# henkkagee/fpc-diffrend

Hardware: AMD Instinct MI355X
Metric: fit-loop frames/sec (9-view 1080p) (higher is better)
Workload: dtype f32; 1 GPU; cfg3: 9-view 1920x1080, K=150 blendshapes, T=30000 triangles, 32 frames/GPU/step (288 images), textured C=1 + antialias fwd/bwd, Adam on weights+pose+texture; frames_per_gpu=32, views=9, triangles=30000, parallelism=one GPU, no collective

## Files before the change

fpc_diffrend_amd/_lib.py:

```python
import ctypes
import os
import subprocess

_HERE = os.path.dirname(os.path.abspath(__file__))
LIB_PATH = os.environ.get("FPCDR_LIB_PATH") or os.path.join(_HERE, "libfpcdr.so")
TWOCALL_LIB_PATH = os.environ.get("FPCDR_TWOCALL_LIB_PATH") or os.path.join(_HERE, "libfpcdr_twocall.so")
CSRC = os.path.join(_HERE, "csrc")

MAX_ATTR = 32
MAX_MIP = 16
LOSS_SLOTS = 256
OCC_BIN = 32
ABI_VERSION = 16

FILTER = {'nearest': 0, 'linear': 1, 'linear-mipmap-nearest': 2, 'linear-mipmap-linear': 3}
BOUNDARY = {'wrap': 0, 'clamp': 1, 'zero': 2}

_p = ctypes.c_void_p
_i = ctypes.c_int32


class RasterizeFwd(ctypes.Structure):
    _fields_ = [("pos", _p), ("tri", _p), ("B", _i), ("V", _i), ("T", _i), ("H", _i), ("W", _i), ("scratch", _p),
                ("rast", _p), ("rast_db", _p), ("hint", _p), ("ranges", _p)]
# ... 99 lines not shown
                ("bg", ctypes.c_float), ("color_scale", ctypes.c_float), ("grad_scale", ctypes.c_float), ("eps", ctypes.c_float),
                ("radius", _i), ("taps", ctypes.c_float * 64), ("tmp", _p), ("stats", _p), ("d", _p), ("pq", _p), ("p", _p),
                ("loss_sum", _p), ("grad_color", _p)]


ROBUST_KIND = {'l2': 0, 'charbonnier': 1, 'geman_mcclure': 2}


class RobustLoss(ctypes.Structure):
    _fields_ = [("color", _p), ("rast", _p), ("ref", _p), ("B", _i), ("H", _i), ("W", _i), ("C", _i),
                ("bg", ctypes.c_float), ("color_scale", ctypes.c_float), ("grad_scale", ctypes.c_float), ("kind", _i),
                ("inv_c", ctypes.c_float), ("w_outside", ctypes.c_float), ("sat", _i), ("mask", _p), ("face_w", _p), ("T", _i),
                ("sums", _p), ("grad_color", _p)]


WSUM_SLOTS = 32


class ObjectiveWeighted(ctypes.Structure):
    _fields_ = [("base", Objective), ("kind", _i), ("inv_c", ctypes.c_float), ("w_outside", ctypes.c_float), ("sat", _i),
                ("T_weights", _i), ("mask", _p), ("face_w", _p), ("wsum", _p)]


ADAM_MAX_TENSORS = 16


class AdamTensor(ctypes.Structure):
    _fields_ = [("param", _p), ("grad", _p), ("exp_avg", _p), ("exp_avg_sq", _p), ("n", ctypes.c_int64),
                ("step_size", ctypes.c_float), ("bc2_sqrt", ctypes.c_float), ("renorm", _i), ("table_row", _i),
                ("step", _i), ("lr", ctypes.c_float)]


class AdamParams(ctypes.Structure):
    _fields_ = [("n_tensors", _i), ("beta1", ctypes.c_float), ("beta2", ctypes.c_float), ("eps", ctypes.c_float),
                ("one_minus_beta1", ctypes.c_float), ("one_minus_beta2", ctypes.c_float), ("t", AdamTensor * ADAM_MAX_TENSORS),
                ("step_table", _p), ("skip_flag", _p), ("skipped", _p), ("lr_skip_gain", ctypes.c_double),
                ("skipped_per_tensor", _p), ("beta1_f64", ctypes.c_double), ("beta2_f64", ctypes.c_double)]


_sz = ctypes.c_size_t
_int = ctypes.c_int
SYMBOLS = {
    "fpcdr_abi_version": (_int, []),
    "fpcdr_last_error": (ctypes.c_char_p, []),
    "fpcdr_rasterize_scratch_bytes": (_sz, [_i, _i]),
    "fpcdr_rasterize_fwd": (_int, [ctypes.POINTER(RasterizeFwd), _p]),
    "fpcdr_rasterize_bwd": (_int, [ctypes.POINTER(RasterizeBwd), _p]),
    "fpcdr_occ_bytes": (_sz, [_i, _i, _i]),
    "fpcdr_cmask_bytes": (_sz, [_i, _i, _i]),
    "fpcdr_objective_cmask_bytes": (_sz, [_i, _i, _i]),
    "fpcdr_ref_bg_sumsq": (_int, [_p, ctypes.c_int64, ctypes.c_int64, ctypes.c_float, _p, _p]),
    "fpcdr_objective_value": (_int, [_p, _i, _p, ctypes.c_double, ctypes.c_double, _p, _p]),
    "fpcdr_idplane_bytes": (_sz, [_i, _i, _i]),
    "fpcdr_binlist_bytes": (_sz, [_i, _i, _i]),
    "fpcdr_objective_fwd": (_int, [ctypes.POINTER(Objective), _p]),
    "fpcdr_silhouette_bits": (_int, [_p, _p, _p, _i, _i, _i, _i, _i, _p, _p]),
    "fpcdr_interpolate_fwd": (_int, [ctypes.POINTER(InterpolateFwd), _p]),
    "fpcdr_interpolate_bwd": (_int, [ctypes.POINTER(InterpolateBwd), _p]),
    "fpcdr_mip_downsample": (_int, [_p, _p, _i, _i, _i, _i, _p]),
    "fpcdr_mip_downsample_bwd": (_int, [_p, _p, _i, _i, _i, _i, _p]),
    "fpcdr_texture_fwd": (_int, [ctypes.POINTER(TextureFwd), _p]),
    "fpcdr_texture_bwd": (_int, [ctypes.POINTER(TextureBwd), _p]),
    "fpcdr_topology_scratch_bytes": (_sz, [_i]),
    "fpcdr_topology_build": (_int, [_p, _i, _p, _p, _p]),
    "fpcdr_antialias_flags_bytes": (_sz, [_i, _i, _i]),
    "fpcdr_antialias_fwd": (_int, [ctypes.POINTER(AntialiasFwd), _p]),
    "fpcdr_antialias_bwd": (_int, [ctypes.POINTER(AntialiasBwd), _p]),
    "fpcdr_transform_clip_fwd": (_int, [_p, _p, _p, _i, _i, _i, _p]),
    "fpcdr_transform_clip_bwd": (_int, [_p, _p, _p, _p, _p, _i, _i, _i, _p]),
    "fpcdr_mvp_fwd": (_int, [_p, _p, _p, _p, _p, _p, _p, _i, _i, _p]),
    "fpcdr_mvp_bwd": (_int, [_p, _p, _p, _p, _p, _p, _p, _p, _p, _p, _p, _i, _i, _p]),
    "fpcdr_mvp_fwd_indexed": (_int, [_p, _p, _p, _p, _p, _p, _p, _p, _p, _p, _i, _i, _p]),
    "fpcdr_mvp_bwd_indexed": (_int, [_p, _p, _p, _p, _p, _p, _p, _p, _p, _p, _p, _p, _p, _p, _i, _i, _p]),
    "fpcdr_laplacian_gather": (_int, [_p, _p, _p, _p, _i, _i, _i, _i, _p]),
    "fpcdr_laplacian_penalty_fwd": (_int, [_p, _p, _p, _p, _p, _p, _p, ctypes.c_float, _i, _i, _i, _p]),
    "fpcdr_laplacian_penalty_bwd": (_int, [_p, _p, _p, _p, _p, _p, ctypes.c_float, _i, _i, _i, _p]),
    "fpcdr_laplacian_penalty_rest_fwd": (_int, [_p, _p, _p, _p, _p, _p, _p, _p, ctypes.c_float, _i, _i, _i, _p]),
    "fpcdr_stretch_penalty": (_int, [_p, _p, _p, ctypes.c_float, _p, _p, _p, _p, ctypes.c_float, _i, _i, _i, _i, _p]),
    "fpcdr_bend_penalty": (_int, [_p, _p, _p, _p, _p, _p, _p, _p, _p, ctypes.c_float, _i, _i, _i, _i, _p]),
    "fpcdr_motion_penalty": (_int, [_p, _p, _p, ctypes.c_float, _i, _p, _p, _p, _p, ctypes.c_float, _i, _i, _p]),
    "fpcdr_tex_prior": (_int, [_p, _p, _p, _p, ctypes.c_float, ctypes.c_float, ctypes.c_float, _p, _p, _p, _p, _i, _i, _i, _p]),
    "fpcdr_blend_fwd": (_int, [_p, _p, _p, _p, _i, _i, _i, _p]),
    "fpcdr_blend_bwd_w": (_int, [_p, _p, _p, _i, _i, _i, _p]),
    "fpcdr_blend_bwd_basis": (_int, [_p, _p, _p, _i, _i, _i, _p]),
    "fpcdr_rig_weights_fwd": (_int, [_p, _p, _p, _i, _i, _i, _i, _i, _p, _p]),
    "fpcdr_rig_weights_bwd": (_int, [_p, _p, _p, _i, _p, _i, _i, _i, _i, _p, _p, _p]),
    "fpcdr_pixel_loss": (_int, [ctypes.POINTER(PixelLoss), _p]),
    "fpcdr_blur_loss_scratch_bytes": (_sz, [_i, _i, _i, _i]),
    "fpcdr_blur_loss": (_int, [ctypes.POINTER(BlurLoss), _p]),
    "fpcdr_norm_loss_scratch_bytes": (_sz, [_i, _i, _i, _i]),
    "fpcdr_norm_loss": (_int, [ctypes.POINTER(NormLoss), _p]),
    "fpcdr_robust_loss": (_int, [ctypes.POINTER(RobustLoss), _p]),
    "fpcdr_objective_weighted_fwd": (_int, [ctypes.POINTER(ObjectiveWeighted), _p]),
    "fpcdr_ref_bg_wsum": (_int, [_p, _p, ctypes.c_int64, ctypes.c_int64, ctypes.c_float, _i, ctypes.c_float, ctypes.c_float, _i, _p, _p]),
    "fpcdr_adam_step": (_int, [ctypes.POINTER(AdamParams), _p]),
    "fpcdr_undistort_u8": (_int, [_p, _p, _p, ctypes.c_int64, _i, _i, _i, _i, _i, _p]),
    "fpcdr_compare_u8": (_int, [_p, _int, ctypes.c_float, _p, _p, _p, ctypes.c_int64, _i, _i, _i, _i, _i, _i, _p]),
    "fpcdr_overlay_u8": (_int, [_p, _int, ctypes.c_float, _p, _p, _p, _p, ctypes.c_int64, _i, _i, _int, _int, ctypes.c_float,
                                ctypes.c_uint32, _int, _p]),
    "fpcdr_bake_accumulate_u8": (_int, [_p, _p, _p, _p, ctypes.c_int64, _i, _i, _i, _i, _i, _i, _i, _p]),
    "fpcdr_bake_resolve": (_int, [_p, _p, _p, _i, _i, ctypes.c_double, ctypes.c_uint64, _p]),
    "fpcdr_bake_dilate": (_int, [_p, _p, _p, _p, _i, _i, _p]),
    "fpcdr_downsample_u8": (_int, [_p, _p, ctypes.c_int64, _i, _i, _i, _p]),
}

SYMBOLS_TWOCALL = {
    "fpcdr_render_fwd": (_int, [ctypes.POINTER(RenderFwd), _p]),
    "fpcdr_render_bwd": (_int, [ctypes.POINTER(RenderBwd), _p]),
    "fpcdr_aa_loss_fwd": (_int, [ctypes.POINTER(AaLossFwd), _p]),
    "fpcdr_render_loss_fwd": (_int, [ctypes.POINTER(RenderFwd), ctypes.POINTER(AaLossFwd), _p, _p]),
    "fpcdr_render_aa_bwd": (_int, [ctypes.POINTER(RenderAaBwd), _p]),
}

_lib = None
_lib_twocall = None


def build(force=False):
    cmd = ["make", "-s", "-C", CSRC, "-j8"] + (["-B"] if force else [])
    subprocess.check_call(cmd)
    return LIB_PATH


def load():
    global _lib
    if _lib is not None:
        return _lib
    if not os.path.exists(LIB_PATH):
        raise RuntimeError(
            f"{LIB_PATH} not found: the HIP extension is not built. Run `python -c 'import __graft_entry__ as g; "
            f"g.build()'` (or `make -C {CSRC}`). There is no CPU fallback for the raster ops.")
    import torch
    hip_rt = os.path.join(os.path.dirname(torch.__file__), "lib", "libamdhip64.so")
    if os.path.exists(hip_rt):
        ctypes.CDLL(hip_rt, mode=ctypes.RTLD_GLOBAL)
    lib = ctypes.CDLL(LIB_PATH)
    for name, (res, args) in SYMBOLS.items():
        fn = getattr(lib, name)
        fn.restype = res
        fn.argtypes = args
    ver = lib.fpcdr_abi_version()
    if ver != ABI_VERSION:
        raise RuntimeError(f"libfpcdr.so ABI version {ver} != binding {ABI_VERSION}; rebuild the extension")
    _lib = lib
    return lib


def load_twocall():
    global _lib_twocall
    if _lib_twocall is not None:
        return _lib_twocall
    load()
    if not os.path.exists(TWOCALL_LIB_PATH):
        raise RuntimeError(f"{TWOCALL_LIB_PATH} not found: run `make -C {CSRC}` (or __graft_entry__.build()). The two-call form of the "
                           "pixel objective and ops.render_textured live in this second library; there is no fallback.")
    lib = ctypes.CDLL(TWOCALL_LIB_PATH)
    for name, (res, args) in list(SYMBOLS.items()) + list(SYMBOLS_TWOCALL.items()):
        fn = getattr(lib, name)
        fn.restype = res
        fn.argtypes = args
    if lib.fpcdr_abi_version() != ABI_VERSION:
        raise RuntimeError(f"libfpcdr_twocall.so ABI version {lib.fpcdr_abi_version()} != binding {ABI_VERSION}; rebuild the extension")
    _lib_twocall = lib
    return lib


# ... 40 lines not shown
```

fpc_diffrend_amd/csrc/blend.hip:

```cpp
#include "common.h"

namespace {

typedef float f32x16 __attribute__((ext_vector_type(16)));

constexpr int KC = 64;

__device__ __forceinline__ int acc_row(int r, int lane) { return (r & 3) + 8 * (r >> 2) + 4 * (lane >> 5); }

__global__ void __launch_bounds__(256) k_blend_fwd(const float *__restrict__ v_base, const float *__restrict__ Bmat,
                                                   const float *__restrict__ w, float *__restrict__ out, int M, int K, int F) {
    const int lane = threadIdx.x & 63, wave = threadIdx.x >> 6;
    const int tile = blockIdx.x * 4 + wave;
    const int i0 = tile * 32;
    if (i0 >= M) return;
    const int col = lane & 31, h = lane >> 5;
    const int row = min(i0 + col, M - 1);
    const float *brow = Bmat + (size_t)row * K;
    for (int f0 = 0; f0 < F; f0 += 32) {
        const int fr = min(f0 + col, F - 1);
        const float *wrow = w + (size_t)fr * K;
        f32x16 acc = {0, 0, 0, 0, 0, 0, 0, 0, 0, 0, 0, 0, 0, 0, 0, 0};
        if ((K & 1) == 0) {
            for (int kc = 0; kc < K; kc += 2 * KC) {
// ... 107 lines not shown
                s_w[r * KP + K + e - r * np] = 0.0f;
            }
        }
        store_tile(s_w, vw4);
        __syncthreads();
        f32x16 acc = {0, 0, 0, 0, 0, 0, 0, 0, 0, 0, 0, 0, 0, 0, 0, 0};
        const float *pa = s_w + col * KP + kbase, *pb = s_b + col * KP + kbase;
        for (int s = 0; s < kh; s += 4) {
            const float4 a = *reinterpret_cast<const float4 *>(pa + s);
            const float4 b = *reinterpret_cast<const float4 *>(pb + s);
            acc = __builtin_amdgcn_mfma_f32_32x32x2f32(a.x, b.x, acc, 0, 0, 0);
            acc = __builtin_amdgcn_mfma_f32_32x32x2f32(a.y, b.y, acc, 0, 0, 0);
            acc = __builtin_amdgcn_mfma_f32_32x32x2f32(a.z, b.z, acc, 0, 0, 0);
            acc = __builtin_amdgcn_mfma_f32_32x32x2f32(a.w, b.w, acc, 0, 0, 0);
        }
        __syncthreads();
        if (wave > 0) {
#pragma unroll
            for (int r = 0; r < 16; ++r) s_red[((wave - 1) * 16 + r) * 64 + lane] = acc[r];
        }
        __syncthreads();
        if (wave == 0) {
            const int i = i0 + col;
            const float vb = (v_base && i < M) ? v_base[i] : 0.0f;
#pragma unroll
            for (int r = 0; r < 16; ++r) {
                const float v = acc[r] + s_red[r * 64 + lane] + s_red[(16 + r) * 64 + lane] + s_red[(32 + r) * 64 + lane];
                const int f = f0 + acc_row(r, lane);
                if (f < F && i < M) out[(size_t)f * M + i] = v + vb;
            }
        }
    }
}

#define FPCDR_BLEND_SLAB 512
constexpr int SLAB = FPCDR_BLEND_SLAB;
__global__ void __launch_bounds__(256) k_blend_bwd_w(const float *__restrict__ Bmat, const float *__restrict__ gout,
                                                     float *__restrict__ grad_w, int M, int K, int F) {
    const int lane = threadIdx.x & 63, wave = threadIdx.x >> 6;
    const int col = lane & 31, h = lane >> 5;
    const int k0 = blockIdx.x * 32, f0 = blockIdx.z * 32;
    const int kk = k0 + col, fr = min(f0 + col, F - 1);
    const int rows_per_wave = SLAB / 4, rows_per_half = rows_per_wave / 2;
    const int base = blockIdx.y * SLAB + wave * rows_per_wave + h * rows_per_half;
    const float *grow = gout + (size_t)fr * M;
    f32x16 acc = {0, 0, 0, 0, 0, 0, 0, 0, 0, 0, 0, 0, 0, 0, 0, 0};
    if ((M & 1) == 0) {
#pragma unroll 8
        for (int s = 0; s < rows_per_half; s += 2) {
            const int i = base + s;
            const bool ok = i < M;
            const float2 a = ok ? *reinterpret_cast<const float2 *>(grow + i) : make_float2(0.f, 0.f);
            const float b0 = (ok && kk < K) ? Bmat[(size_t)i * K + kk] : 0.0f;
            const float b1 = (ok && kk < K) ? Bmat[(size_t)(i + 1) * K + kk] : 0.0f;
            acc = __builtin_amdgcn_mfma_f32_32x32x2f32(a.x, b0, acc, 0, 0, 0);
            acc = __builtin_amdgcn_mfma_f32_32x32x2f32(a.y, b1, acc, 0, 0, 0);
        }
    } else {
#pragma unroll 8
        for (int s = 0; s < rows_per_half; ++s) {
            const int i = base + s;
            const bool ok = i < M;
            const float a = ok ? grow[i] : 0.0f;
            const float b = (ok && kk < K) ? Bmat[(size_t)i * K + kk] : 0.0f;
            acc = __builtin_amdgcn_mfma_f32_32x32x2f32(a, b, acc, 0, 0, 0);
        }
    }
    __shared__ float s_red[3][16][64];
    if (wave > 0) {
#pragma unroll
        for (int r = 0; r < 16; ++r) s_red[wave - 1][r][lane] = acc[r];
    }
    __syncthreads();
    if (wave == 0 && kk < K) {
#pragma unroll
        for (int r = 0; r < 16; ++r) {
            const int f = f0 + acc_row(r, lane);
            const float v = acc[r] + s_red[0][r][lane] + s_red[1][r][lane] + s_red[2][r][lane];
            if (f < F && v != 0.0f) atomicAdd(grad_w + (size_t)f * K + kk, v);
        }
    }
}

__global__ void __launch_bounds__(256) k_blend_bwd_basis(const float *__restrict__ w, const float *__restrict__ gout,
                                                         float *__restrict__ grad_B, int M, int K, int F) {
    const int lane = threadIdx.x & 63, wave = threadIdx.x >> 6;
    const int col = lane & 31, h = lane >> 5;
    const int i0 = (blockIdx.x * 4 + wave) * 32, k0 = blockIdx.y * 32;
    if (i0 >= M) return;
    const int ii = min(i0 + col, M - 1), kk = min(k0 + col, K - 1);
    f32x16 acc = {0, 0, 0, 0, 0, 0, 0, 0, 0, 0, 0, 0, 0, 0, 0, 0};
    const int half = (F + 1) / 2;
    for (int s = 0; s < half; ++s) {
        const int f = h * half + s;
        const bool ok = f < F && (h == 0 ? s < half : true);
        const float a = ok ? gout[(size_t)f * M + ii] : 0.0f;
        const float b = ok ? w[(size_t)f * K + kk] : 0.0f;
        acc = __builtin_amdgcn_mfma_f32_32x32x2f32(a, b, acc, 0, 0, 0);
    }
    const int k = k0 + col;
    if (k < K) {
#pragma unroll
        for (int r = 0; r < 16; ++r) {
            const int i = i0 + acc_row(r, lane);
            if (i < M) grad_B[(size_t)i * K + k] = acc[r];
        }
    }
}

__device__ __forceinline__ int rig_col(const int64_t *__restrict__ cols, int col0, int fb, int Fc) {
    if (!cols) return col0 + fb;
    long long c = cols[fb];
    if (c < 0) c += Fc;
    return (c >= 0 && c < Fc) ? (int)c : -1;
}

__global__ void __launch_bounds__(256) k_rig_weights_fwd(const float *__restrict__ mi, const float *__restrict__ maps,
                                                         const int64_t *__restrict__ cols, int col0, int K, int Fr, int Fc, int Fb,
                                                         float *__restrict__ w) {
    const int idx = blockIdx.x * 256 + threadIdx.x;
    if (idx >= Fb * K) return;
    const int fb = idx / K, k = idx - fb * K;
    const int c = rig_col(cols, col0, fb, Fc);
    if (c < 0) { w[idx] = __int_as_float(0x7fc00000); return; }
    float s = 0.0f;
#pragma unroll 8
    for (int f = 0; f < Fr; ++f) s += mi[(size_t)k * Fr + f] * maps[(size_t)f * Fc + c];
    w[idx] = s;
}

__global__ void __launch_bounds__(256) k_rig_weights_bwd(const float *__restrict__ mi, const float *__restrict__ maps,
                                                         const int64_t *__restrict__ cols, int col0, const float *__restrict__ g_w,
                                                         int K, int Fr, int Fc, int Fb, float *__restrict__ g_mi, float *__restrict__ g_maps) {
    const int lane = threadIdx.x & 63;
    int idx = blockIdx.x * 4 + (threadIdx.x >> 6);
    if (idx < K * Fr) {
        if (!g_mi) return;
        const int k = idx / Fr, f = idx - k * Fr;
        float s = 0.0f;
        for (int fb = lane; fb < Fb; fb += 64) {
            const int c = rig_col(cols, col0, fb, Fc);
            if (c >= 0) s += g_w[(size_t)fb * K + k] * maps[(size_t)f * Fc + c];
        }
        s = wave_sum_dpp(s);
        if (lane == 0) g_mi[idx] = s;
        return;
    }
    idx -= K * Fr;
    if (idx >= Fr * Fc || !g_maps) return;
    const int f = idx / Fc, c = idx - f * Fc;
    float s = 0.0f;
    for (int fb = 0; fb < Fb; ++fb) {
        if (rig_col(cols, col0, fb, Fc) != c) continue;
        for (int k = lane; k < K; k += 64) s += mi[(size_t)k * Fr + f] * g_w[(size_t)fb * K + k];
    }
    s = wave_sum_dpp(s);
    if (lane == 0) g_maps[idx] = s;
}

}

extern "C" int fpcdr_blend_fwd(const float *v_base, const float *Bmat, const float *w, float *out, int32_t M, int32_t K,
                               int32_t F, void *stream) {
    FPCDR_REQUIRE(Bmat && w && out, "null pointer");
    FPCDR_REQUIRE(M > 0 && K > 0 && F > 0, "sizes must be positive");
    if (K <= LDS_KMAX && ((size_t)Bmat & 15) == 0 && ((size_t)w & 15) == 0) {
        const int KQ = (K + 31) / 32 * 32;
        const size_t tile = (size_t)32 * (KQ + 4);
        const size_t lds = (tile + (tile > 3 * 16 * 64 ? tile : (size_t)3 * 16 * 64)) * sizeof(float);
        hipLaunchKernelGGL(k_blend_fwd_lds, dim3(fpcdr_cdiv(M, TM)), dim3(256), lds, (hipStream_t)stream, v_base, Bmat, w, out, M, K,
                           F, KQ);
        FPCDR_CHECK_LAUNCH();
        return FPCDR_OK;
    }
    hipLaunchKernelGGL(k_blend_fwd, dim3(fpcdr_cdiv(fpcdr_cdiv(M, 32), 4)), dim3(256), 0, (hipStream_t)stream, v_base, Bmat, w,
                       out, M, K, F);
    FPCDR_CHECK_LAUNCH();
    return FPCDR_OK;
}

extern "C" int fpcdr_blend_bwd_w(const float *Bmat, const float *grad_out, float *grad_w, int32_t M, int32_t K, int32_t F,
                                 void *stream) {
    FPCDR_REQUIRE(Bmat && grad_out && grad_w, "null pointer");
    FPCDR_REQUIRE(M > 0 && K > 0 && F > 0, "sizes must be positive");
    FPCDR_REQUIRE(fpcdr_cdiv(M, SLAB) <= 65535 && fpcdr_cdiv(F, 32) <= 65535, "problem too large for one launch");
    dim3 grid(fpcdr_cdiv(K, 32), fpcdr_cdiv(M, SLAB), fpcdr_cdiv(F, 32));
    hipLaunchKernelGGL(k_blend_bwd_w, grid, dim3(256), 0, (hipStream_t)stream, Bmat, grad_out, grad_w, M, K, F);
    FPCDR_CHECK_LAUNCH();
    return FPCDR_OK;
}

extern "C" int fpcdr_blend_bwd_basis(const float *w, const float *grad_out, float *grad_B, int32_t M, int32_t K, int32_t F,
                                     void *stream) {
    FPCDR_REQUIRE(w && grad_out && grad_B, "null pointer");
    FPCDR_REQUIRE(M > 0 && K > 0 && F > 0, "sizes must be positive");
    FPCDR_REQUIRE(fpcdr_cdiv(K, 32) <= 65535, "K too large for one launch");
    dim3 grid(fpcdr_cdiv(fpcdr_cdiv(M, 32), 4), fpcdr_cdiv(K, 32));
    hipLaunchKernelGGL(k_blend_bwd_basis, grid, dim3(256), 0, (hipStream_t)stream, w, grad_out, grad_B, M, K, F);
    FPCDR_CHECK_LAUNCH();
    return FPCDR_OK;
}

extern "C" int fpcdr_rig_weights_fwd(const float *mi, const float *maps, const int64_t *cols, int32_t col0, int32_t K, int32_t Fr, int32_t Fc,
                                     int32_t Fb, float *w, void *stream) {
    FPCDR_REQUIRE(mi && maps && w, "null pointer");
    FPCDR_REQUIRE(K > 0 && Fr > 0 && Fc > 0 && Fb > 0 && (long long)Fb * K < (1ll << 30), "bad sizes");
    FPCDR_REQUIRE(cols || (col0 >= 0 && col0 + Fb <= Fc), "column range outside maps");
    hipLaunchKernelGGL(k_rig_weights_fwd, dim3(fpcdr_cdiv(Fb * K, 256)), dim3(256), 0, (hipStream_t)stream, mi, maps, cols, col0, K, Fr, Fc, Fb, w);
    FPCDR_CHECK_LAUNCH();
    return FPCDR_OK;
}

extern "C" int fpcdr_rig_weights_bwd(const float *mi, const float *maps, const int64_t *cols, int32_t col0, const float *grad_w, int32_t K,
                                     int32_t Fr, int32_t Fc, int32_t Fb, float *grad_mi, float *grad_maps, void *stream) {
    FPCDR_REQUIRE(mi && maps && grad_w, "null pointer");
    FPCDR_REQUIRE(K > 0 && Fr > 0 && Fc > 0 && Fb > 0 && (long long)Fb * K < (1ll << 30) && (long long)K * Fr + (long long)Fr * Fc < (1ll << 30),
                  "bad sizes");
    FPCDR_REQUIRE(cols || (col0 >= 0 && col0 + Fb <= Fc), "column range outside maps");
    hipLaunchKernelGGL(k_rig_weights_bwd, dim3(fpcdr_cdiv(K * Fr + Fr * Fc, 4)), dim3(256), 0, (hipStream_t)stream, mi, maps, cols, col0,
                       grad_w, K, Fr, Fc, Fb, grad_mi, grad_maps);
    FPCDR_CHECK_LAUNCH();
    return FPCDR_OK;
}
```

fpc_diffrend_amd/fit.py:

```python
import ctypes
import json
import math
import os
import time
from dataclasses import dataclass
from typing import Optional, Sequence, Tuple

import numpy as np
import torch

from . import _lib, camera
from . import ops as dr
from .mesh_reg import (MeshTopology, RestShape, _check_item_weights, _uniform_laplacian, bend_penalty, check_motion_options,
                       hinge_incidence, hinge_rest_cs, hinge_vertices, laplacian_penalty, mesh_edge_loss, mesh_laplacian_smoothing,
                       mesh_normal_consistency, motion_inv_scale, motion_penalty, rest_edge_lengths, stretch_penalty)
from .ops import _ptr, _stream
from .tex_prior import chart_map, check_tex_prior_options, load_texel_weights, tex_prior_inv_scale, texture_prior

BACKGROUND = 45.0 / 255.0



class ZeroPool:

    def __init__(self, buf=None):
        self.buf, self.off = buf, 0

    def zeros(self, shape, device):
        n = int(np.prod(shape))
        if self.buf is not None and self.buf.device == device and self.off + n <= self.buf.numel():
            v = self.buf[self.off:self.off + n].view(shape)
            self.off += (n + 3) // 4 * 4
            return v
        return torch.zeros(shape, dtype=torch.float32, device=device)


def _pool_zeros(pool, shape, device):
    return pool.zeros(shape, device) if pool is not None else torch.zeros(shape, dtype=torch.float32, device=device)


class _blend_func(torch.autograd.Function):

    @staticmethod
    def forward(ctx, v_base, Bmat, w, pool=None):
        lib = _lib.load()
        M, K = Bmat.shape
        F = w.shape[0]
        out = torch.empty(F, M, dtype=torch.float32, device=w.device)
        _lib.call("fpcdr_blend_fwd", _ptr(v_base), _ptr(Bmat), _ptr(w), _ptr(out), M, K, F, _stream())
        ctx.save_for_backward(Bmat, w)
        ctx.pool = pool
        return out

    @staticmethod
    def backward(ctx, g):
        lib = _lib.load()
        Bmat, w = ctx.saved_tensors
        M, K = Bmat.shape
        F = w.shape[0]
        g = g.contiguous()
        g_vb = g.sum(dim=0) if ctx.needs_input_grad[0] else None
        g_B = None
        if ctx.needs_input_grad[1]:
            g_B = torch.empty_like(Bmat)
            _lib.call("fpcdr_blend_bwd_basis", _ptr(w), _ptr(g), _ptr(g_B), M, K, F, _stream())
        g_w = None
        if ctx.needs_input_grad[2]:
            g_w = _pool_zeros(ctx.pool, tuple(w.shape), w.device)
            _lib.call("fpcdr_blend_bwd_w", _ptr(Bmat), _ptr(g), _ptr(g_w), M, K, F, _stream())
        return g_vb, g_B, g_w, None


class _transform_clip_func(torch.autograd.Function):

    @staticmethod
    def forward(ctx, mvp, verts, pool=None):
        B, F, V = mvp.shape[0], verts.shape[0], verts.shape[1]
        out = torch.empty(B, V, 4, dtype=torch.float32, device=verts.device)
        _lib.call("fpcdr_transform_clip_fwd", _ptr(mvp), _ptr(verts), _ptr(out), F, B // F, V, _stream())
        ctx.save_for_backward(mvp, verts)
        ctx.pool = pool
        return out

    @staticmethod
    def backward(ctx, g):
        mvp, verts = ctx.saved_tensors
        B, F, V = mvp.shape[0], verts.shape[0], verts.shape[1]
        g = g.contiguous()
        g_mvp = _pool_zeros(ctx.pool, tuple(mvp.shape), mvp.device) if ctx.needs_input_grad[0] else None
        g_verts = torch.empty_like(verts) if ctx.needs_input_grad[1] else None
        _lib.call("fpcdr_transform_clip_bwd", _ptr(mvp), _ptr(verts), _ptr(g), _ptr(g_verts), _ptr(g_mvp), F, B // F, V, _stream())
        return g_mvp, g_verts, None


class _rig_weights_func(torch.autograd.Function):

    @staticmethod
    def forward(ctx, mi, maps, ids, validate=True):
        K, Fr = mi.shape
        Fc = maps.shape[1]
        if isinstance(ids, slice):
            lo, hi, step = ids.indices(Fc)
            assert step == 1
            cols, col0, Fb = None, lo, hi - lo
        else:
            cols, col0, Fb = ids.to(torch.int64).contiguous(), 0, int(ids.shape[0])
            if validate and Fb and bool(((cols < -Fc) | (cols >= Fc)).any()):
                raise IndexError(f"rig_weights: frame index out of range for {Fc} columns")
        w = torch.empty(Fb, K, dtype=torch.float32, device=mi.device)
        _lib.call("fpcdr_rig_weights_fwd", _ptr(mi), _ptr(maps), _ptr(cols), col0, K, Fr, Fc, Fb, _ptr(w), _stream())
        ctx.save_for_backward(mi, maps, *([cols] if cols is not None else []))
        ctx.geom = (col0, K, Fr, Fc, Fb, cols is not None)
        return w

    @staticmethod
    def backward(ctx, g):
        col0, K, Fr, Fc, Fb, has_cols = ctx.geom
        mi, maps = ctx.saved_tensors[:2]
        cols = ctx.saved_tensors[2] if has_cols else None
        g_mi = torch.empty_like(mi) if ctx.needs_input_grad[0] else None
        g_maps = torch.empty_like(maps) if ctx.needs_input_grad[1] else None
        _lib.call("fpcdr_rig_weights_bwd", _ptr(mi), _ptr(maps), _ptr(cols), col0, _ptr(g.contiguous()), K, Fr, Fc, Fb, _ptr(g_mi), _ptr(g_maps),
                  _stream())
        return g_mi, g_maps, None, None


def rig_weights(mi, maps, ids, validate=True):
    if mi.is_cuda and mi.dtype == torch.float32 and mi.is_contiguous() and maps.is_contiguous() and \
            not (isinstance(ids, slice) and ids.step not in (None, 1)):
        return _rig_weights_func.apply(mi, maps, ids, validate)
    return torch.matmul(mi, maps[:, ids]).t()


def transform_clip_batched(mvp, verts, pool=None):
    assert mvp.shape[0] % verts.shape[0] == 0
    return _transform_clip_func.apply(mvp.contiguous(), verts.contiguous(), pool)


def blend_batched(v_base, Bmat, w, pool=None):
    return _blend_func.apply(v_base.contiguous() if v_base is not None else None, Bmat.contiguous(), w.contiguous(), pool)


def _frame_matrix(frames):
    return frames if frames.dim() == 2 else frames[:, None]


def blend(v_base, maps, maps_intermediate, dataset, frames):
    fm = _frame_matrix(frames)
    mapped = torch.matmul(maps['local'], fm)
    if 'global' not in dataset:
        mapped = torch.matmul(maps_intermediate['local'], mapped)
    out = blend_batched(v_base, dataset['local'], mapped.t())
# ... 1398 lines not shown
```

include/fpcdr.h:

```cpp
#ifndef FPCDR_H
#define FPCDR_H

#include <stddef.h>
#include <stdint.h>

#ifdef __cplusplus
extern "C" {
#endif

#define FPCDR_ABI_VERSION 16

enum {
    FPCDR_OK = 0,
    FPCDR_EINVAL = 1,
    FPCDR_ELAUNCH = 2
};

int fpcdr_abi_version(void);
const char *fpcdr_last_error(void);


#define FPCDR_HINT_BYTES(B, H, W) ((size_t)2 * (B) * FPCDR_OCC_DIM(H) * FPCDR_OCC_DIM(W))

size_t fpcdr_rasterize_scratch_bytes(int32_t B, int32_t T);
// ... 176 lines not shown
typedef struct {
    const float *color;
    const float *rast;
    const float *pos;
    const int32_t *tri;
    const int32_t *adj;
    int32_t B, H, W, C, V, T;
    uint8_t *sil;
    uint64_t *flags;
    float *out;
    const uint8_t *hint;
    const float *empty_color;
} fpcdr_antialias_fwd_params;
int fpcdr_antialias_fwd(const fpcdr_antialias_fwd_params *p, void *stream);

typedef struct {
    const float *color, *rast, *pos;
    const int32_t *tri, *adj;
    const float *dy;
    int32_t B, H, W, C, V, T;
    const uint8_t *sil;
    const uint64_t *flags;
    float pos_gradient_boost;
    float *grad_color;
    float *grad_pos;
} fpcdr_antialias_bwd_params;
int fpcdr_antialias_bwd(const fpcdr_antialias_bwd_params *p, void *stream);


int fpcdr_transform_clip_fwd(const float *mvp, const float *verts, float *out, int32_t F, int32_t Nc, int32_t V, void *stream);
int fpcdr_transform_clip_bwd(const float *mvp, const float *verts, const float *grad_out, float *grad_verts, float *grad_mvp,
                             int32_t F, int32_t Nc, int32_t V, void *stream);

int fpcdr_mvp_fwd(const float *proj, const float *t_mv, const float *q_cam, const float *t_cam, const float *q_frame,
                  const float *t_frame, float *mvp, int32_t Fb, int32_t Nc, void *stream);
int fpcdr_mvp_bwd(const float *proj, const float *t_mv, const float *q_cam, const float *t_cam, const float *q_frame,
                  const float *t_frame, const float *grad_mvp, float *gq_cam, float *gt_cam, float *gq_frame, float *gt_frame,
                  int32_t Fb, int32_t Nc, void *stream);
int fpcdr_mvp_fwd_indexed(const float *proj, const float *t_mv, const float *q_cam, const float *t_cam, const float *q_frame,
                          const float *t_frame, const int64_t *frame_idx, const int64_t *view_idx, const int64_t *cam_of_view, float *mvp,
                          int32_t Fb, int32_t Nc, void *stream);
int fpcdr_mvp_bwd_indexed(const float *proj, const float *t_mv, const float *q_cam, const float *t_cam, const float *q_frame,
                          const float *t_frame, const int64_t *frame_idx, const int64_t *view_idx, const int64_t *cam_of_view,
                          const float *grad_mvp, float *gq_cam, float *gt_cam, float *gq_frame, float *gt_frame, int32_t Fb, int32_t Nc,
                          void *stream);


int fpcdr_laplacian_gather(const float *x, const int32_t *nbr, const float *inv_deg, float *out, int32_t F, int32_t V, int32_t D,
                           int32_t transpose, void *stream);

int fpcdr_laplacian_penalty_fwd(const float *x, const int32_t *nbr, const float *inv_deg, float *lap, void *acc, float *per, float *out,
                                float weight, int32_t F, int32_t V, int32_t D, void *stream);
int fpcdr_laplacian_penalty_bwd(const float *lap, const int32_t *nbr, const float *inv_deg, const float *per, const float *upstream,
                                float *grad_x, float weight, int32_t F, int32_t V, int32_t D, void *stream);

int fpcdr_laplacian_penalty_rest_fwd(const float *x, const int32_t *nbr, const float *inv_deg, const float *rest_lap ,
                                     float *lap, void *acc, float *per, float *out, float weight, int32_t F, int32_t V, int32_t D,
                                     void *stream);

int fpcdr_stretch_penalty(const float *x, const int32_t *nbr, const float *rest_len , float target,
                          float *grad_x , void *acc ,
                          float *per, float *out, float weight, int32_t F, int32_t V, int32_t D, int32_t E, void *stream);

int fpcdr_bend_penalty(const float *x, const int32_t *hinge_vtx, const float *rest_cs , const int32_t *hinge_inc,
                       float *hinge_grad , float *grad_x ,
                       void *acc , float *per, float *out, float weight, int32_t F, int32_t V,
                       int32_t H, int32_t K, void *stream);

int fpcdr_motion_penalty(const float *x, const int64_t *frame_t , const float *vertex_w ,
                         float inv_c , int32_t order, float *grad_x ,
                         void *acc , float *per, float *out, float weight, int32_t F, int32_t V,
                         void *stream);

int fpcdr_tex_prior(const float *tex, const float *anchor , const float *smooth_w ,
                    const float *anchor_w , float inv_c , float w_smooth, float w_anchor,
                    float *grad_tex , void *acc , float *part ,
                    float *out, int32_t Ht, int32_t Wt, int32_t C, void *stream);


int fpcdr_blend_fwd(const float *v_base, const float *Bmat, const float *w, float *out, int32_t M, int32_t K,
                    int32_t F, void *stream);
int fpcdr_blend_bwd_w(const float *Bmat, const float *grad_out, float *grad_w, int32_t M, int32_t K, int32_t F,
                      void *stream);
int fpcdr_blend_bwd_basis(const float *w, const float *grad_out, float *grad_B, int32_t M, int32_t K, int32_t F,
                          void *stream);

int fpcdr_rig_weights_fwd(const float *mi, const float *maps, const int64_t *cols, int32_t col0, int32_t K, int32_t Fr, int32_t Fc,
                          int32_t Fb, float *w, void *stream);
int fpcdr_rig_weights_bwd(const float *mi, const float *maps, const int64_t *cols, int32_t col0, const float *grad_w, int32_t K,
                          int32_t Fr, int32_t Fc, int32_t Fb, float *grad_mi, float *grad_maps, void *stream);


typedef struct {
    const float *color;
    const float *rast;
    const uint8_t *ref;
    int32_t B, H, W, C;
    float bg;
    float color_scale;
    float grad_scale;
    double *loss_sum;
    float *grad_color;
} fpcdr_pixel_loss_params;
int fpcdr_pixel_loss(const fpcdr_pixel_loss_params *p, void *stream);


#define FPCDR_ADAM_MAX_TENSORS 16
typedef struct {
    float *param;
    const float *grad;
    float *exp_avg;
    float *exp_avg_sq;
    int64_t n;
    float step_size;
    float bc2_sqrt;
    int32_t renorm;
    int32_t table_row;
    int32_t step;
    float lr;
} fpcdr_adam_tensor;
typedef struct {
    int32_t n_tensors;
    float beta1, beta2, eps;
    float one_minus_beta1, one_minus_beta2;
    fpcdr_adam_tensor t[FPCDR_ADAM_MAX_TENSORS];
    const float *step_table;
    const float *skip_flag;
    int32_t *skipped;
    double lr_skip_gain;
    int32_t *skipped_per_tensor;
    double beta1_f64, beta2_f64;
} fpcdr_adam_params;
int fpcdr_adam_step(const fpcdr_adam_params *p, void *stream);

int fpcdr_undistort_u8(const uint8_t *src, uint8_t *dst, const double *cam_table, int64_t n_images, int H, int W, int n_cam,
                       int clip_max, int flip_rows, void *stream);

int fpcdr_compare_u8(const void *img, int img_is_float, float scale, const uint8_t *ref, uint8_t *heat, int32_t *row_sums,
                     int64_t n_images, int H, int W, int col0, int col1, int mode, int flip_rows, void *stream);

int fpcdr_overlay_u8(const void *img, int img_is_float, float scale, const uint8_t *ref, const float *rast, const float *rast_db,
                     uint8_t *out, int64_t n_images, int H, int W, int weight_256, int outside_capture, float wire_hw2,
                     uint32_t wire_rgb, int flip_rows, void *stream);

typedef struct fpcdr_blur_loss_params fpcdr_blur_loss_params;
struct fpcdr_blur_loss_params {
    const float *color;
    const float *rast;
    const uint8_t *ref;
    int32_t B, H, W, C;
    float bg;
    float color_scale;
    float grad_scale;
    int32_t radius;
    float taps[64];
    float *tmp;
    float *blurred;
    double *loss_sum;
    float *grad_color;
};
size_t fpcdr_blur_loss_scratch_bytes(int32_t B, int32_t H, int32_t W, int32_t C);
int fpcdr_blur_loss(const fpcdr_blur_loss_params *p, void *stream);

int fpcdr_bake_accumulate_u8(const float *texc, const float *rast, const uint8_t *ref, uint64_t *acc, int64_t n_images, int H, int W,
                             int Ht, int Wt, int boundary_mode, int interior_only, int flip_rows, void *stream);
int fpcdr_bake_resolve(const uint64_t *acc, float *tex, uint8_t *filled, int Ht, int Wt, double color_scale, uint64_t min_den,
// ... 76 lines not shown
```

Measured before the change: 13930 frames/s.

## Compute blend weight gradient with slab partial sums instead of atomics

Adds a workspace-based path for the blendshape weight gradient. Each workgroup owns a slab of rows and stages the basis and output-gradient chunks in LDS with register prefetch, accumulating across all K tiles with MFMA. It writes per-slab partial results, which a second kernel reduces deterministically into grad_w. This is meant to remove the per-element atomicAdd contention and repeated global loads of the old kernel, at the cost of a per-call workspace allocation, an extra launch and extra partial-sum memory traffic.

```diff
diff --git a/fpc_diffrend_amd/_lib.py b/fpc_diffrend_amd/_lib.py
--- a/fpc_diffrend_amd/_lib.py
+++ b/fpc_diffrend_amd/_lib.py
@@ -205,6 +205,8 @@
     "fpcdr_tex_prior": (_int, [_p, _p, _p, _p, ctypes.c_float, ctypes.c_float, ctypes.c_float, _p, _p, _p, _p, _i, _i, _i, _p]),
     "fpcdr_blend_fwd": (_int, [_p, _p, _p, _p, _i, _i, _i, _p]),
     "fpcdr_blend_bwd_w": (_int, [_p, _p, _p, _i, _i, _i, _p]),
+    "fpcdr_blend_bwd_w_workspace_bytes": (_sz, [_i, _i, _i]),
+    "fpcdr_blend_bwd_w_ws": (_int, [_p, _p, _p, _p, _sz, _i, _i, _i, _p]),
     "fpcdr_blend_bwd_basis": (_int, [_p, _p, _p, _i, _i, _i, _p]),
     "fpcdr_rig_weights_fwd": (_int, [_p, _p, _p, _i, _i, _i, _i, _i, _p, _p]),
     "fpcdr_rig_weights_bwd": (_int, [_p, _p, _p, _i, _p, _i, _i, _i, _i, _p, _p, _p]),
diff --git a/fpc_diffrend_amd/csrc/blend.hip b/fpc_diffrend_amd/csrc/blend.hip
--- a/fpc_diffrend_amd/csrc/blend.hip
+++ b/fpc_diffrend_amd/csrc/blend.hip
@@ -213,6 +213,150 @@
     }
 }
 
+constexpr int WS_WGS = 256;
+static int ws_slab_rows(int M) { return fpcdr_cdiv(fpcdr_cdiv(M, WS_WGS) < 1 ? 1 : fpcdr_cdiv(M, WS_WGS), 64) * 64; }
+
+template <int KT>
+__global__ void __launch_bounds__(256) k_blend_bwd_w_slab(const float *__restrict__ Bmat, const float *__restrict__ gout,
+                                                          float *__restrict__ part, int M, int K, int F, int slab_rows) {
+    constexpr int RC = KT <= 6 ? 64 : 32;
+    constexpr int GS = RC + 1;
+    constexpr int NQB = RC * KT / 32;
+    constexpr int NQF = RC / 4 + 1;
+    constexpr int NQG = (32 * NQF + 255) / 256;
+    extern __shared__ float smem[];
+    float *s_b = smem;
+    float *s_g = smem + ((RC * K + 32 + 3) & ~3);
+    float *s_red = smem;
+    const int tid = threadIdx.x, lane = tid & 63, wave = tid >> 6;
+    const int col = lane & 31, h = lane >> 5;
+    const int slab0 = blockIdx.x * slab_rows, slab_end = min(slab0 + slab_rows, M);
+    const int f0 = blockIdx.y * 32;
+    const long long total = (long long)F * M;
+    const int n4 = RC * K / 4;
+    float4 vb[NQB], vg[NQG];
+    auto load_chunk = [&](int r0) {
+        const float *__restrict__ src = Bmat + (size_t)r0 * K;
+        const int nb = min(RC, slab_end - r0) * K;
+#pragma unroll
+        for (int j = 0; j < NQB; ++j) {
+            const int q = tid + 256 * j, e0 = 4 * q;
+            vb[j] = make_float4(0.f, 0.f, 0.f, 0.f);
+            if (q < n4) {
+                if (e0 + 3 < nb) vb[j] = *reinterpret_cast<const float4 *>(src + e0);
+                else {
+                    if (e0 < nb) vb[j].x = src[e0];
+                    if (e0 + 1 < nb) vb[j].y = src[e0 + 1];
+                    if (e0 + 2 < nb) vb[j].z = src[e0 + 2];
+                }
+            }
+        }
+#pragma unroll
+        for (int j = 0; j < NQG; ++j) {
+            const int idx = tid + 256 * j, f = idx / NQF, q = idx - f * NQF;
+            vg[j] = make_float4(0.f, 0.f, 0.f, 0.f);
+            if (f < 32 && f0 + f < F) {
+                const long long e0 = (((long long)(f0 + f) * M + r0) & ~3ll) + 4 * q;
+                if (e0 + 3 < total) vg[j] = *reinterpret_cast<const float4 *>(gout + e0);
+                else {
+                    if (e0 < total) vg[j].x = gout[e0];
+                    if (e0 + 1 < total) vg[j].y = gout[e0 + 1];
+                    if (e0 + 2 < total) vg[j].z = gout[e0 + 2];
+                }
+            }
+        }
+    };
+    auto store_chunk = [&](int r0) {
+        const int rows = min(RC, slab_end - r0);
+#pragma unroll
+        for (int j = 0; j < NQB; ++j) {
+            const int q = tid + 256 * j;
+            if (q < n4) *reinterpret_cast<float4 *>(s_b + 4 * q) = vb[j];
+        }
+#pragma unroll
+        for (int j = 0; j < NQG; ++j) {
+            const int idx = tid + 256 * j, f = idx / NQF, q = idx - f * NQF;
+            if (f < 32) {
+                const int r = 4 * q - (int)(((long long)(f0 + f) * M + r0) & 3ll);
+                const float vv[4] = {vg[j].x, vg[j].y, vg[j].z, vg[j].w};
+#pragma unroll
+                for (int c = 0; c < 4; ++c)
+                    if (r + c >= 0 && r + c < RC) s_g[f * GS + r + c] = r + c < rows ? vv[c] : 0.0f;
+            }
+        }
+    };
+    f32x16 acc[KT];
+#pragma unroll
+    for (int t = 0; t < KT; ++t) acc[t] = f32x16{0, 0, 0, 0, 0, 0, 0, 0, 0, 0, 0, 0, 0, 0, 0, 0};
+    const int rbase = wave * (RC / 4) + h * (RC / 8);
+    load_chunk(slab0);
+    for (int r0 = slab0; r0 < slab_end; r0 += RC) {
+        store_chunk(r0);
+        __syncthreads();
+        if (r0 + RC < slab_end) load_chunk(r0 + RC);
+#pragma unroll
+        for (int s = 0; s < RC / 8; ++s) {
+            const float a = s_g[col * GS + rbase + s];
+            const float *pb = s_b + (rbase + s) * K + col;
+#pragma unroll
+            for (int t = 0; t < KT; ++t) acc[t] = __builtin_amdgcn_mfma_f32_32x32x2f32(a, pb[32 * t], acc[t], 0, 0, 0);
+        }
+        __syncthreads();
+    }
+    for (int w = 1; w < 4; ++w) {
+        if (wave == w) {
+#pragma unroll
+            for (int t = 0; t < KT; ++t)
+#pragma unroll
+                for (int r = 0; r < 16; ++r) s_red[(t * 16 + r) * 64 + lane] = acc[t][r];
+        }
+        __syncthreads();
+        if (wave == 0) {
+#pragma unroll
+            for (int t = 0; t < KT; ++t)
+#pragma unroll
+                for (int r = 0; r < 16; ++r) acc[t][r] += s_red[(t * 16 + r) * 64 + lane];
+        }
+        __syncthreads();
+    }
+    if (wave == 0) {
+        float *__restrict__ dst = part + (size_t)blockIdx.x * F * K;
+#pragma unroll
+        for (int t = 0; t < KT; ++t) {
+            const int k = 32 * t + col;
+#pragma unroll
+            for (int r = 0; r < 16; ++r) {
+                const int f = f0 + acc_row(r, lane);
+                if (f < F && k < K) dst[(size_t)f * K + k] = acc[t][r];
+            }
+        }
+    }
+}
+
+__global__ void __launch_bounds__(256) k_blend_bwd_w_sum(const float *__restrict__ part, float *__restrict__ grad_w, int nslabs, int n) {
+    __shared__ float s_p[16][17];
+    const int tid = threadIdx.x, j = tid & 15, g = tid >> 4;
+    const int e = blockIdx.x * 16 + j;
+    float s = 0.0f;
+    if (e < n) {
+        for (int s0 = g; s0 < nslabs; s0 += 256) {
+            float v[16];
+#pragma unroll
+            for (int u = 0; u < 16; ++u) v[u] = s0 + 16 * u < nslabs ? part[(size_t)(s0 + 16 * u) * n + e] : 0.0f;
+#pragma unroll
+            for (int u = 0; u < 16; ++u) s += v[u];
+        }
+    }
+    s_p[g][j] = s;
+    __syncthreads();
+    if (tid < 16 && e < n) {
+        float t = s_p[0][tid];
+#pragma unroll
+        for (int i = 1; i < 16; ++i) t += s_p[i][tid];
+        grad_w[e] += t;
+    }
+}
+
 __global__ void __launch_bounds__(256) k_blend_bwd_basis(const float *__restrict__ w, const float *__restrict__ gout,
                                                          float *__restrict__ grad_B, int M, int K, int F) {
     const int lane = threadIdx.x & 63, wave = threadIdx.x >> 6;
@@ -321,6 +465,45 @@
     return FPCDR_OK;
 }
 
+extern "C" size_t fpcdr_blend_bwd_w_workspace_bytes(int32_t M, int32_t K, int32_t F) {
+    if (M <= 0 || K <= 0 || F <= 0) return 0;
+    return (size_t)fpcdr_cdiv(M, ws_slab_rows(M)) * (size_t)F * (size_t)K * sizeof(float);
+}
+
+template <int KT>
+static void launch_bwd_w_slab(const float *Bmat, const float *grad_out, float *part, int M, int K, int F, int slab_rows, hipStream_t st) {
+    constexpr int RC = KT <= 6 ? 64 : 32;
+    const size_t chunk = (size_t)((RC * K + 32 + 3) & ~3) + 32 * (RC + 1), red = (size_t)KT * 16 * 64;
+    hipLaunchKernelGGL(k_blend_bwd_w_slab<KT>, dim3(fpcdr_cdiv(M, slab_rows), fpcdr_cdiv(F, 32)), dim3(256),
+                       (chunk > red ? chunk : red) * sizeof(float), st, Bmat, grad_out, part, M, K, F, slab_rows);
+}
+
+extern "C" int fpcdr_blend_bwd_w_ws(const float *Bmat, const float *grad_out, float *grad_w, void *workspace, size_t workspace_bytes,
+                                    int32_t M, int32_t K, int32_t F, void *stream) {
+    FPCDR_REQUIRE(Bmat && grad_out && grad_w, "null pointer");
+    FPCDR_REQUIRE(M > 0 && K > 0 && F > 0, "sizes must be positive");
+    FPCDR_REQUIRE(!workspace || workspace_bytes >= fpcdr_blend_bwd_w_workspace_bytes(M, K, F), "workspace too small");
+    if (!workspace || K > LDS_KMAX || (((size_t)Bmat | (size_t)grad_out | (size_t)workspace) & 15) != 0 || fpcdr_cdiv(F, 32) > 65535 ||
+        (long long)F * K >= (1ll << 30))
+        return fpcdr_blend_bwd_w(Bmat, grad_out, grad_w, M, K, F, stream);
+    const int slab_rows = ws_slab_rows(M), nslabs = fpcdr_cdiv(M, slab_rows);
+    float *part = (float *)workspace;
+    hipStream_t st = (hipStream_t)stream;
+    switch (fpcdr_cdiv(K, 32)) {
+    case 1: launch_bwd_w_slab<1>(Bmat, grad_out, part, M, K, F, slab_rows, st); break;
+    case 2: launch_bwd_w_slab<2>(Bmat, grad_out, part, M, K, F, slab_rows, st); break;
+    case 3: launch_bwd_w_slab<3>(Bmat, grad_out, part, M, K, F, slab_rows, st); break;
+    case 4: launch_bwd_w_slab<4>(Bmat, grad_out, part, M, K, F, slab_rows, st); break;
+    case 5: launch_bwd_w_slab<5>(Bmat, grad_out, part, M, K, F, slab_rows, st); break;
+    case 6: launch_bwd_w_slab<6>(Bmat, grad_out, part, M, K, F, slab_rows, st); break;
+    default: launch_bwd_w_slab<7>(Bmat, grad_out, part, M, K, F, slab_rows, st); break;
+    }
+    FPCDR_CHECK_LAUNCH();
+    hipLaunchKernelGGL(k_blend_bwd_w_sum, dim3(fpcdr_cdiv((long long)F * K, 16)), dim3(256), 0, st, part, grad_w, nslabs, F * K);
+    FPCDR_CHECK_LAUNCH();
+    return FPCDR_OK;
+}
+
 extern "C" int fpcdr_blend_bwd_basis(const float *w, const float *grad_out, float *grad_B, int32_t M, int32_t K, int32_t F,
                                      void *stream) {
     FPCDR_REQUIRE(w && grad_out && grad_B, "null pointer");
diff --git a/fpc_diffrend_amd/fit.py b/fpc_diffrend_amd/fit.py
--- a/fpc_diffrend_amd/fit.py
+++ b/fpc_diffrend_amd/fit.py
@@ -67,7 +67,8 @@
         g_w = None
         if ctx.needs_input_grad[2]:
             g_w = _pool_zeros(ctx.pool, tuple(w.shape), w.device)
-            _lib.call("fpcdr_blend_bwd_w", _ptr(Bmat), _ptr(g), _ptr(g_w), M, K, F, _stream())
+            ws = torch.empty(lib.fpcdr_blend_bwd_w_workspace_bytes(M, K, F) // 4, dtype=torch.float32, device=w.device)
+            _lib.call("fpcdr_blend_bwd_w_ws", _ptr(Bmat), _ptr(g), _ptr(g_w), _ptr(ws), ws.numel() * 4, M, K, F, _stream())
         return g_vb, g_B, g_w, None
 
 
diff --git a/include/fpcdr.h b/include/fpcdr.h
--- a/include/fpcdr.h
+++ b/include/fpcdr.h
@@ -282,6 +282,9 @@
                     int32_t F, void *stream);
 int fpcdr_blend_bwd_w(const float *Bmat, const float *grad_out, float *grad_w, int32_t M, int32_t K, int32_t F,
                       void *stream);
+size_t fpcdr_blend_bwd_w_workspace_bytes(int32_t M, int32_t K, int32_t F);
+int fpcdr_blend_bwd_w_ws(const float *Bmat, const float *grad_out, float *grad_w, void *workspace, size_t workspace_bytes,
+                         int32_t M, int32_t K, int32_t F, void *stream);
 int fpcdr_blend_bwd_basis(const float *w, const float *grad_out, float *grad_B, int32_t M, int32_t K, int32_t F,
                           void *stream);
 
```

New measurement: 14160 frames/s, median of 6. 1.02x the previous value.
